# qiyu3816/DiffSG

Hardware: AMD Instinct MI355X
Metric: ddpm_reverse_sample_steps_per_sec_msr80c (higher is better)
Workload: dtype f32(2xf16-split MFMA, f32 accumulate); 1 GPU; MSR-80c CFG reverse sampling, batch 65536 x D=C=80 per GPU, UNet1D(proj 128, dims (64,32,16,8), n_blocks 2), omega=1, device Philox noise; rows sharded, no collective; batch_per_gpu=65536, solution_dim=80, parallelism=rows x1

## Files before the change

diffsg_amd/UNetCF.py:

```python
from __future__ import annotations

import ctypes

import torch
import torch.nn as nn

from . import _lib


class _ParamsOnly(nn.Module):
    def forward(self, *a, **k):
        raise RuntimeError("parameter holder: the arithmetic lives in libdiffsg_hip.so (call UNet1D.forward)")


class TimeEmbedding(_ParamsOnly):

    def __init__(self, in_dim):
        super().__init__()
        self.in_dim = in_dim
        self.lin1 = nn.Linear(in_dim // 4, in_dim)
        self.lin2 = nn.Linear(in_dim, in_dim)


class ResidualBlock(_ParamsOnly):
# ... 231 lines not shown
    def set_precision(self, mode):
        code = {"split_f16": 0, "f32": 1}[mode]
        for hd in self._all_handles():
            _lib.check(_lib.lib().dsg_set_precision(hd, code))
        self.__dict__.setdefault("_settings", {})["precision"] = code

    @property
    def precision(self):
        return {0: "split_f16", 1: "f32"}[self.__dict__.get("_settings", {}).get("precision", 0)]

    def range_exceeded(self):
        hit = False
        for nat in [self._native] + list(self.__dict__.get("_twins", {}).values()):
            hd = nat.handle
            if hd is None:
                continue
            flag = ctypes.c_int(0)
            with torch.cuda.device(self._named_param_list()[0][1].device):
                _lib.check(_lib.lib().dsg_range_status_stream(hd, ctypes.byref(flag), _lib.stream_ptr()))
            hit = hit or bool(flag.value)
        return hit

    def check_range(self):
        if self.range_exceeded():
            raise RuntimeError("libdiffsg_hip: an activation exceeded the fp16 range of the split-f16 path (|x| > 6e4); "
                               "the results of the last calls are invalid -- use set_precision('f32') for this model")

    def set_launch_policy(self, coop_max_tiles=-1, narrow_small_max_tiles=-1):
        for hd in self._all_handles():
            _lib.check(_lib.lib().dsg_set_launch_policy(hd, int(coop_max_tiles), int(narrow_small_max_tiles)))
        self.__dict__.setdefault("_settings", {})["policy"] = (int(coop_max_tiles), int(narrow_small_max_tiles))

    def set_option(self, name, value):
        code = {"narrow_valu8": 1, "train_time_beside": 2, "wgrad_narrow_part": 4, "tile_step": 8, "panel_half": 16, "f32_pair": 32}[name]
        for hd in self._all_handles():
            _lib.check(_lib.lib().dsg_set_option(hd, code, int(value)))
        self.__dict__.setdefault("_settings", {}).setdefault("options", {})[code] = int(value)

    def _all_handles(self):
        return [self.native_handle()] + [self.native_handle(k) for k in self.__dict__.get("_twins", {})]

    def forward(self, x, t, cond, cond_mask):
        hd = self.native_handle()
        B = x.shape[0]
        x = x.detach().to(torch.float32).contiguous()
        cond = cond.detach().to(torch.float32).contiguous()
        tv = t.detach().to(torch.float32).reshape(-1).contiguous()
        mk = cond_mask.detach().to(torch.float32).reshape(-1).contiguous()
        if tv.numel() != B or mk.numel() != B or cond.shape[0] != B:
            raise ValueError("t, cond and cond_mask must have one entry per row of x")
        if x.shape[1] != self.cfg["input_dim"] or cond.shape[1] != self.cfg["cond_dim"]:
            raise ValueError("x / cond feature size does not match the model")
        out = torch.empty_like(x)
        if B == 0:
            return out
        with torch.cuda.device(x.device):
            _lib.check(_lib.lib().dsg_unet_forward(hd, _lib.ptr(x), _lib.ptr(tv), _lib.ptr(cond), _lib.ptr(mk),
                                                   _lib.ptr(out), B, _lib.stream_ptr()))
        return out
```

diffsg_amd/csrc/dsg_api.hip:

```cpp
#include "dsg_kernels.hpp"
#include "dsg_train.hpp"
#include "dsg_split.hpp"
#include "dsg_wide.hpp"
#include "dsg_panel.hpp"
#include "dsg_res64.hpp"
#include "dsg_tile.hpp"
#include "dsg_train_split.hpp"
#include "dsg_eval.hpp"
#include "dsg_labelgen.hpp"
#include "dsg_cogen.hpp"
#include "dsg_nugen.hpp"
#include "../../include/diffsg.h"

#include <math.h>
#include <stdarg.h>
#include <stdio.h>
#include <string.h>

#include <string>
#include <algorithm>
#include <vector>

using namespace dsg;

// ... 141 lines not shown
    int device = 0;
    int* range_flag = nullptr;
    int* range_pinned = nullptr;
    CallParams* call_dev = nullptr;
    hipStream_t cap_stream = nullptr;
    std::vector<double> op_ms;
    bool train_prof = false;
    hipEvent_t tev[6] = {nullptr, nullptr, nullptr, nullptr, nullptr, nullptr};
    bool tev_valid = false;
    std::vector<int> op_calls;

    int fuse_lo = 0, fuse_hi = 0;
    FusedOp* fused_dev = nullptr;
    std::vector<FusedOp> fused_host;
    FusedOpH* fusedh_dev = nullptr;
    FusedOpH* tileops_dev = nullptr;
    std::vector<FusedOpH> tileops_host;
    bool tile_valid = false, opt_tile = true;
    bool opt_panel_half = true;
    FusedOpH* fusedh_train_dev = nullptr;
    const void* fusedh_train_key[4] = {nullptr, nullptr, nullptr, nullptr}; int fusedh_train_rows = 0;
    struct FusedSig { bool valid = false, sp = false, share = false; int nrows = 0, npass = 0, uncond_tiles = 0; const void* p[8] = {}; } fused_sig;
    FusedOp* ce_dev = nullptr;
    std::vector<FusedOp> ce_host;
    CondTile* ctile_dev = nullptr; int ctile_n = 0; const float* ctile_key = nullptr; size_t ctile_cap = 0;
    std::vector<FusedOpH> fusedh_host;
    NarrowLdsOp* nlds_ops_dev = nullptr; NarrowLdsCopy* nlds_copies_dev = nullptr; uint4* nlds_image = nullptr;
    std::vector<NarrowPhaseArgs> nlds_phases;
    bool nlds_tail = false;
    bool nlds_valid = false;
    int v8_lo = -1, v8_hi = -1;
    bool opt_v8 = true;
    bool opt_f32_pair = true;
    bool opt_time_beside = true;
    bool opt_wg_narrow_part = false;
    float* v8_image = nullptr; NarrowLdsCopy* v8_copies_dev = nullptr; int v8_ncopies = 0;
    int nlds_ncopies = 0;
    size_t nlds_image_cap = 0;

    hipGraphExec_t gexec[1 + 6] = {};
    int g_rows = -1, g_chunks = -1, g_chunk_rows = -1;
    unsigned long long* seeds_dev = nullptr; int seeds_cap = 0;
    double* red_chunks = nullptr; int red_chunks_cap = 0;

    size_t tr_per_tile = 0;
    size_t tr_yt_frag = 0, tr_deps = 0;
    int tr_rows = 0, tr_T = 0, tr_chunks = 0;
    float* tr_ws = nullptr;
    float* tr_slabs = nullptr;
    float* tr_gsum = nullptr;
    unsigned* tr_gmax = nullptr;
    unsigned* tr_gmax_t = nullptr;
    int gmax_ld = 0;
    float* tr_cs = nullptr;
    int4* cs_map_dev = nullptr;
    int cs_slots = 0;
    int n_gmax = 0;
    size_t slab_stride = 0;
    int* tr_ts = nullptr;
    float* tr_noise = nullptr; float* tr_mask = nullptr;
    float* tr_yt_rm = nullptr;
    float* tr_tsave = nullptr;
    long long* tw_dst_dev = nullptr; const float** tw_src_dev = nullptr; int tw_rows = 0;
    WgradDesc* wg_desc_dev = nullptr; WgradUnit* wg_unit_dev = nullptr; int wg_units = 0;
    std::vector<int> wg_forks = {3, 6};
    std::vector<int> wg_part_end;
// ... 396 lines not shown
    }
}

void fill_block_args_h(const dsg_handle* h, const ResP& r, const BlockArgs& b, BlockArgsH& a) {
    a.b = b;
    const float* A = h->arena;
    a.W1h = reinterpret_cast<const uint4*>(A + r.W1h); a.W2h = reinterpret_cast<const uint4*>(A + r.W2h);
    a.W3h = reinterpret_cast<const uint4*>(A + r.W3h); a.Wsch = r.sclin ? reinterpret_cast<const uint4*>(A + r.Wsch) : nullptr;
    a.m1 = h->maxabs + r.l1.w; a.m2 = h->maxabs + r.l2.w; a.m3 = h->maxabs + r.l3.w; a.msc = r.sclin ? h->maxabs + r.sc.w : nullptr;
    a.kc = h->opc_dev + 4 * (size_t)(&r - h->res.data());
}
void fill_lin_args_h(const dsg_handle* h, const LinOpP& l, const LinArgs& b, LinArgsH& a) {
    a.l = b;
    a.Wh = reinterpret_cast<const uint4*>(h->arena + l.Wh);
    a.m = h->maxabs + l.l.w;
    a.kc = h->opc_dev + 4 * (h->res.size() + (size_t)(&l - h->lin.data()));
}

template <int N>
void launch_res_h_n(bool sclin, const BlockArgsH& a, hipStream_t s) {
    const dim3 grid(cdiv(a.b.ntiles, kWavesPerBlock)), block(256);
    if (sclin) hipLaunchKernelGGL((k_resblock_h<N, true>), grid, block, 0, s, a);
    else hipLaunchKernelGGL((k_resblock_h<N, false>), grid, block, 0, s, a);
}

bool wide128_ok(const ResP& r, const BlockArgs& b) {
    return r.N == 128 && b.in0.groups == 16 && (b.in1.groups == 0 || b.in1.groups == 16) && (b.in1.groups != 0) == r.sclin && b.cond_pre;
}

bool panel128_ok(const dsg_handle* h, const ResP& r, const BlockArgs& b) {
    return wide128_ok(r, b) && !b.ts && !b.save_h1 && b.tiles_per_pass * 2 >= b.ntiles && b.ntiles >= h->panel_min_tiles &&
           b.ntiles > h->coop_max_tiles;
}
template <bool SC, int EPI, int NTO>
void launch_panel128(const dsg_handle* h, const BlockLinArgsH& w, hipStream_t s) {
    if (h->opt_panel_half) {
        const int ngroups = cdiv(w.b.b.ntiles, 4);
        const dim3 grid(ngroups < 2 * h->num_cus ? ngroups : 2 * h->num_cus), block(256);
        hipLaunchKernelGGL((k_panel128_h<SC, EPI, NTO, 2>), grid, block, 0, s, w, ngroups);
        return;
    }
    const int ngroups = cdiv(w.b.b.ntiles, kPW);
    const dim3 grid(ngroups < h->num_cus ? ngroups : h->num_cus), block(kPW * 64);
    hipLaunchKernelGGL((k_panel128_h<SC, EPI, NTO>), grid, block, 0, s, w, ngroups);
}

bool res64_lds_ok(const dsg_handle* h, const ResP& r, const BlockArgs& b) {
    return r.N == 64 && b.in0.groups == 8 && (b.in1.groups == 0 || b.in1.groups == 8) && (b.in1.groups != 0) == r.sclin && b.cond_pre && !b.ts &&
           !b.save_h1 && b.tiles_per_pass * 2 >= b.ntiles && b.ntiles >= h->panel_min_tiles && b.ntiles > h->coop_max_tiles;
}

void launch_res_h(const dsg_handle* h, const ResP& r, const BlockArgs& b, hipStream_t s) {
    BlockArgsH a;
    fill_block_args_h(h, r, b, a);
    const int ks1 = (groups_of(r.in0) + 1) / 2 + (groups_of(r.in1) + 1) / 2;
    const bool coop_fits = ks1 * 128 <= kCoopLdsU4 / (4 / (r.N / 32 > 0 ? r.N / 32 : 1)) / 2 && r.in0 == r.N && r.in1 == (r.sclin ? r.N : 0);
    const int coop_max = (a.b.save_h1 && h->coop_max_tiles > 0 && h->coop_max_tiles < kCoopMaxTilesTrain) ? kCoopMaxTilesTrain : h->coop_max_tiles;
    if ((r.N == 64 || r.N == 128) && coop_fits && a.b.ntiles <= coop_max) {
        const int tpw = 4 / (r.N / 32);
        const dim3 grid(cdiv(a.b.ntiles, tpw)), block(256);
        if (r.N == 128) {
            if (r.sclin) hipLaunchKernelGGL((k_resblock_c<128, true>), grid, block, 0, s, a);
            else hipLaunchKernelGGL((k_resblock_c<128, false>), grid, block, 0, s, a);
        } else {
            if (r.sclin) hipLaunchKernelGGL((k_resblock_c<64, true>), grid, block, 0, s, a);
            else hipLaunchKernelGGL((k_resblock_c<64, false>), grid, block, 0, s, a);
        }
        return;
    }
    if (res64_lds_ok(h, r, a.b)) {
        const int ngroups = cdiv(a.b.ntiles, kR64Waves);
        const dim3 grid(ngroups < h->num_cus ? ngroups : h->num_cus), block(kR64Waves * 64);
        BlockLinArgsH w;
        memset(&w, 0, sizeof w);
        w.b = a; w.store_block_out = 1;
        if (r.sclin) hipLaunchKernelGGL((k_res64_lds<true, 0>), grid, block, 0, s, w, ngroups);
        else hipLaunchKernelGGL((k_res64_lds<false, 0>), grid, block, 0, s, w, ngroups);
// ... 62 lines not shown
    }
    if (panel128_ok(h, r, b) && l.l.K == 128) {
#define DSG_TRYP(SC_, EPI_, NTO_)                                                                            \
    if (r.sclin == SC_ && (final_op ? 2 : 1) == EPI_ && NTO == NTO_) {                                       \
        launch_panel128<SC_, EPI_, NTO_>(h, a, s);                                                           \
        return true;                                                                                         \
    }
        DSG_TRYP(false, 1, 2) DSG_TRYP(false, 1, 1) DSG_TRYP(true, 2, 1) DSG_TRYP(true, 2, 3)
#undef DSG_TRYP
    }
    if (wide128_ok(r, b) && l.l.K == 128) {
#define DSG_TRYW(SC_, EPI_, NTO_)                                                                            \
    if (r.sclin == SC_ && (final_op ? 2 : 1) == EPI_ && NTO == NTO_) {                                       \
        hipLaunchKernelGGL((k_wide128_h<SC_, EPI_, NTO_>), grid, block, 0, s, a);                            \
        return true;                                                                                         \
    }
        DSG_TRYW(false, 1, 2) DSG_TRYW(false, 1, 1) DSG_TRYW(true, 2, 1) DSG_TRYW(true, 2, 3)
#undef DSG_TRYW
    }
#define DSG_TRY(N_, SC_, NTO_, FIN_)                                                                         \
    if (r.N == N_ && r.sclin == SC_ && NTO == NTO_ && final_op == FIN_) {                                    \
        hipLaunchKernelGGL((k_resblock_lin_h<N_, SC_, NTO_, FIN_>), grid, block, 0, s, a);                   \
        return true;                                                                                         \
    }
    DSG_TRY(128, false, 2, false) DSG_TRY(128, false, 1, false) DSG_TRY(64, true, 4, false) DSG_TRY(64, false, 2, false)
    DSG_TRY(64, true, 2, false) DSG_TRY(64, false, 1, false)
    DSG_TRY(128, true, 1, true) DSG_TRY(128, true, 3, true) DSG_TRY(64, true, 1, true) DSG_TRY(64, true, 3, true)
#undef DSG_TRY
    return false;
}

bool split_ctx(const dsg_handle* h, const RunCtx& c) { return h->use_split && c.cond_pre; }

void launch_op(const dsg_handle* h, const Op& op, const RunCtx& c, hipStream_t s) {
    if (op.kind == OP_RES) {
        BlockArgs a;
        fill_block_args(h, op, c, a);
        const ResP& r = h->res[op.p];
        if (split_ctx(h, c)) launch_res_h(h, r, a, s);
        else launch_res(r.N, r.sclin, a, s);
    } else {
        LinArgs a;
        fill_lin_args(h, op, c, a);
        const int inmode = op.kind == OP_PROJ ? IN_ROWMAJOR : IN_FRAG;
        const int outmode = op.kind == OP_FINAL ? OUT_ROWMAJOR : OUT_FRAG;
        if (split_ctx(h, c)) {
            LinArgsH ah;
            fill_lin_args_h(h, h->lin[op.p], a, ah);
            launch_lin_h(h->lin[op.p].l.N, inmode, outmode, op.kind == OP_FINAL, ah, s);
        } else {
            launch_lin(h->lin[op.p].l.N, inmode, outmode, op.kind == OP_FINAL, a, s);
        }
    }
}

bool fusable(const dsg_handle* h, const Op& op) {
    if (op.kind == OP_RES) return h->res[op.p].N <= 32;
    if (op.kind == OP_LIN) return h->lin[op.p].l.N <= 32;
    return false;
}

int prepare_fused(dsg_handle* h, const RunCtx& c, hipStream_t s) {
    const int n = h->fuse_hi - h->fuse_lo;
    if (n < 2) return 0;
    const bool sp = split_ctx(h, c);
    if (c.train) {
        if (!sp) return 0;
        const void* key[4] = {h->ws, h->tr_ws, h->cembed, h->tb};
        if (h->fusedh_train_dev && h->fusedh_train_rows == c.nrows && !memcmp(key, h->fusedh_train_key, sizeof key)) return 0;
        if (!h->fusedh_train_dev) HIPCK(hipMalloc(&h->fusedh_train_dev, (h->ops.size() + 1) * sizeof(FusedOpH)));
        memcpy(h->fusedh_train_key, key, sizeof key);
        h->fusedh_train_rows = c.nrows;
// ... 1169 lines not shown
    DeviceGuard dg(h);
    if (mode != DSG_PRECISION_SPLIT_F16 && mode != DSG_PRECISION_F32_MFMA) return fail("unknown precision mode %d", mode);
    const bool split = mode == DSG_PRECISION_SPLIT_F16;
    if (split != h->use_split) { (void)hipDeviceSynchronize(); free_graphs(h); h->use_split = split; }
    return 0;
}

int dsg_set_renorm_hook(dsg_handle* h, double* stats3, void (*reduce)(void*), void* user) {
    if (!h) return fail("null handle");
    if (reduce && !stats3) return fail("dsg_set_renorm_hook: a reduce function needs the 3-double device buffer");
    h->renorm_stats = stats3; h->renorm_fn = reduce; h->renorm_user = user;
    return 0;
}

int dsg_set_option(dsg_handle* h, int option, int value) {
    if (!h) return fail("null handle");
    DeviceGuard dg(h);
    switch (option) {
        case DSG_OPT_NARROW_VALU8:
            if ((value != 0) != h->opt_v8) {
                (void)hipDeviceSynchronize();
                free_graphs(h);
                h->fused_sig.valid = false;
                h->opt_v8 = value != 0;
            }
            return 0;
        case DSG_OPT_TRAIN_TIME_BESIDE: h->opt_time_beside = value != 0; return 0;
        case DSG_OPT_PANEL_HALF:
            if ((value != 0) != h->opt_panel_half) { (void)hipDeviceSynchronize(); free_graphs(h); h->opt_panel_half = value != 0; }
            return 0;
        case DSG_OPT_F32_PAIR:
            if ((value != 0) != h->opt_f32_pair) { (void)hipDeviceSynchronize(); free_graphs(h); h->opt_f32_pair = value != 0; }
            return 0;
        case DSG_OPT_TILE_STEP:
            if ((value != 0) != h->opt_tile) { (void)hipDeviceSynchronize(); free_graphs(h); h->opt_tile = value != 0; }
            return 0;
        case DSG_OPT_WGRAD_NARROW_PART:
            if ((value != 0) != h->opt_wg_narrow_part) { (void)hipDeviceSynchronize(); h->opt_wg_narrow_part = value != 0; h->td_valid = false; }
            return 0;
        default: return fail("dsg_set_option: unknown option %d", option);
    }
}

int dsg_range_status(dsg_handle* h, int* exceeded) {
    if (!h || !exceeded) return fail("dsg_range_status: null argument");
    DeviceGuard dg(h);
    HIPCK(hipDeviceSynchronize());
    HIPCK(hipMemcpy(exceeded, h->range_flag, sizeof(int), hipMemcpyDeviceToHost));
    if (*exceeded) HIPCK(hipMemset(h->range_flag, 0, sizeof(int)));
    return 0;
}

int dsg_range_status_stream(dsg_handle* h, int* exceeded, void* stream) {
    if (!h || !exceeded) return fail("dsg_range_status_stream: null argument");
    DeviceGuard dg(h);
    hipStream_t s = (hipStream_t)stream;
    if (!h->range_pinned) HIPCK(hipHostMalloc(reinterpret_cast<void**>(&h->range_pinned), sizeof(int), hipHostMallocDefault));
    hipLaunchKernelGGL(k_flag_take, dim3(1), dim3(64), 0, s, h->range_flag, h->range_pinned);
    HIPCK(hipGetLastError());
    HIPCK(hipStreamSynchronize(s));
    *exceeded = *h->range_pinned;
    return 0;
}

int dsg_set_launch_policy(dsg_handle* h, int coop_max_tiles, int narrow_small_max_tiles) {
    if (!h) return fail("null handle");
// ... 793 lines not shown
```

diffsg_amd/csrc/dsg_panel.hpp:

```cpp
#pragma once
#include "dsg_wide.hpp"

namespace dsg {

constexpr int kPW = 8;
constexpr int kPanelU4 = 2048;
constexpr int kPrivU4 = 128;
constexpr int kPrivSlots = 5;
constexpr int kPrivDist = 4;
constexpr int kPanelLdsU4 = 2 * kPanelU4 + kPW * kPrivSlots * kPrivU4 + kWideVec / 4;
constexpr int panel_pw(int steps) { return 2 * steps; }
constexpr int panel_u4(int steps) { return 512 * steps; }
constexpr int panel_lds_u4(int steps) { return 2 * panel_u4(steps) + panel_pw(steps) * kPrivSlots * kPrivU4 + kWideVec / 4; }

#ifndef DSG_STAMP_DBG
#define DSG_STAMP_DBG 0
#endif
#ifdef DSG_CYCLE_STAMPS
constexpr int kPanelStampU4 = kPW * 128 / 2;
#define DSG_PSTAMP(tag)                                                                                               \
    do {                                                                                                              \
        if (STAMPED && blockIdx.x == 0 && stamp_k < 128) {                                                           \
            const unsigned long long t_ = __builtin_readcyclecounter();                                               \
            if (lane == 0 && !(DSG_STAMP_DBG & 1)) stamp_lds[wave * 128 + stamp_k] = (t_ << 16) | (unsigned long long)(tag); \
// ... 216 lines not shown
        const int S = j < NJ ? S0 + 1 + j : nx.S, q = m & 3, tt = (S >> 1) & 3, r0 = 8 * (S & 1) + 2 * q, hs = m >> 1, e = 2 * (m & 1);
        const float dcur = j < NJ ? dd : ddn;
        if (ph == 0) {
            const float x0 = MEM ? xq[hs][e] : (j < NJ ? in[tt][r0] : (*nx.in)[tt][r0]), x1 = MEM ? xq[hs][e + 1] : (j < NJ ? in[tt][r0 + 1] : (*nx.in)[tt][r0 + 1]);
            if (LN) {
                u0 = fmaf(fmaf(x0, cp, dcur), gq[hs][e], bq[hs][e]);
                u1 = fmaf(fmaf(x1, cp, dcur), gq[hs][e + 1], bq[hs][e + 1]);
                p0 = __builtin_amdgcn_exp2f(u0); p1 = __builtin_amdgcn_exp2f(u1);
            } else {
                u0 = x0 * (cp * kRawScale); u1 = x1 * (cp * kRawScale);
            }
        } else if (ph == 1) {
            if (LN) {
                v0 = u0 * __builtin_amdgcn_rcpf(fmaf(p0, kk, kk));
                v1 = u1 * __builtin_amdgcn_rcpf(fmaf(p1, kk, kk));
            } else { v0 = u0; v1 = u1; }
        } else {
            unsigned a, er;
            split_pair_nowait(v0, v1, a, er);
            hq[m] = __builtin_bit_cast(float, a); lq[m] = __builtin_bit_cast(float, er);
        }
    }
    if (HASN) {
        constexpr int L0 = 4 * NJ;
        asm volatile("" : "+v"(hq[L0 + 3]), "+v"(lq[L0 + 3]));
        const f32x4 hv = {hq[L0], hq[L0 + 1], hq[L0 + 2], hq[L0 + 3]}, lv = {lq[L0], lq[L0 + 1], lq[L0 + 2], lq[L0 + 3]};
        bcarry.hi = __builtin_bit_cast(h8, hv); bcarry.lo = __builtin_bit_cast(h8, lv);
    }
}

#ifndef DSG_PANEL_TRAIL_PRIO
#define DSG_PANEL_TRAIL_PRIO 1
#endif
template <bool SCLIN, int EPI, int NTO, int STEPS = 4>
__global__ __launch_bounds__(64 * panel_pw(STEPS), 2) void k_panel128_h(const BlockLinArgsH A, const int ngroups) {
    constexpr int N = 128, NT = 4, NG = 16;
    constexpr int PW = panel_pw(STEPS), PU4 = panel_u4(STEPS), NTHR = 64 * PW;
    constexpr int KS1 = SCLIN ? 16 : 8, P1 = KS1 / STEPS, P2 = 8 / STEPS, NE = SCLIN ? 16 : 8;
    constexpr int NTOP = NTO <= 1 ? 1 : (NTO == 2 ? 2 : 4), ESTEPS = 4 * STEPS / NTOP;
    constexpr int EPANELS = EPI == 0 ? 0 : (ESTEPS >= 8 ? 1 : 8 / ESTEPS);
    constexpr int PA = P1, PB = PA + P2, PD = PB + P2, PE = PD + (SCLIN ? P1 : 0), NP = PE + EPANELS;
    __shared__ uint4 lds[panel_lds_u4(STEPS) + (STEPS == 4 ? kPanelStampU4 : 0)];
#ifdef DSG_CYCLE_STAMPS
    unsigned long long* const stamp_lds = reinterpret_cast<unsigned long long*>(lds + panel_lds_u4(STEPS));
    int stamp_k = 0;
    constexpr bool STAMPED = SCLIN && EPI == 0 && STEPS == 4;
#endif
    float* const vec = reinterpret_cast<float*>(lds + 2 * PU4 + PW * kPrivSlots * kPrivU4);
    float* const g1v = vec, * const b1v = vec + kLnLdsW1, * const v2 = vec + 2 * kLnLdsW1;
    float* const g2v = v2, * const b2v = v2 + 128, * const g3v = v2 + 256, * const b3v = v2 + 384, * const tbv = v2 + 512, * const c2v = v2 + 640,
         * const c3v = v2 + 768, * const gLv = v2 + 896, * const bLv = v2 + 1024, * const biasLv = v2 + 1152;
    const BlockArgsH& ah = A.b;
    const BlockArgs& a = ah.b;
    const int lane = threadIdx.x & 63, h = lane >> 5, j = lane & 31;
    const int wave = __builtin_amdgcn_readfirstlane(threadIdx.x >> 6);
    const int stride = gridDim.x;
#ifdef DSG_CYCLE_STAMPS
    const unsigned long long clk_t0 = __builtin_readcyclecounter(), clk_r0 = __builtin_amdgcn_s_memrealtime();
#endif
    const bool lead = wave < 4;
    if (STEPS == 4 && !lead) __builtin_amdgcn_s_setprio(DSG_PANEL_TRAIL_PRIO);
    constexpr float kL2 = -1.44269504088896341f;

    {
        const int n1 = ln1_extent(a);
        for (int i = threadIdx.x; i < n1; i += NTHR) { g1v[i] = a.gamma1[i] * kL2; b1v[i] = a.beta1[i] * kL2; }
        if (threadIdx.x < 128) {
            const int i = threadIdx.x;
            g2v[i] = a.gamma2[i] * kL2; b2v[i] = a.beta2[i] * kL2; g3v[i] = a.gamma3[i] * kL2; b3v[i] = a.beta3[i] * kL2;
            c2v[i] = a.c2[i]; c3v[i] = a.c3[i];
            tbv[i] = a.tbias[(size_t)(a.step_ptr ? *a.step_ptr : 0) * a.tb_stride + i];
            if (EPI == 2) { gLv[i] = A.l.l.gamma[i] * kL2; bLv[i] = A.l.l.beta[i] * kL2; }
            if (EPI != 0) biasLv[i] = i < NTO * 32 ? A.l.l.bias[i] : 0.f;
        }
    }
    const float inv1 = ah.kc[0], inv2 = ah.kc[1], inv3 = ah.kc[2];
    float invL = 0.f;
    if (EPI != 0) invL = A.l.kc[EPI == 2 ? 1 : 0];
    __syncthreads();

    const int wnt = wave / (STEPS / 2), wsub = wave % (STEPS / 2);
    const uint4* const w1p = ah.W1h + ((size_t)wnt * KS1) * 128 + wsub * 256;
    const uint4* const w2p = ah.W2h + ((size_t)wnt * 8) * 128 + wsub * 256;
    const uint4* const w3p = ah.W3h + ((size_t)wnt * 8) * 128 + wsub * 256;
    const uint4* const wsp = SCLIN ? ah.Wsch + ((size_t)wnt * KS1) * 128 + wsub * 256 : w1p;
    const uint4* wlp = w1p;
    if (EPI != 0) {
        if (NTOP == 4) wlp = A.l.Wh + ((size_t)(wnt < NTO ? wnt : 0) * 8) * 128 + wsub * 256;
        else if (NTOP == 2) wlp = A.l.Wh + ((size_t)(wave / STEPS) * 8) * 128 + (wave % STEPS) * 256;
        else wlp = A.l.Wh + (wave & 3) * 256;
    }
    auto panel_src = [&](int p) -> const uint4* {
        if (p < PA) return w1p + (size_t)p * (128 * STEPS);
        if (p < PB) return w2p + (size_t)(p - PA) * (128 * STEPS);
        if (p < PD) return w3p + (size_t)(p - PB) * (128 * STEPS);
        if (p < PE) return wsp + (size_t)(p - PD) * (128 * STEPS);
        return wlp + (ESTEPS < 8 ? (size_t)(p - PE) * (128 * ESTEPS) : 0);
    };

    const unsigned lds0 = (unsigned)(unsigned long long)(const __attribute__((address_space(3))) void*)lds;
    PanelCtx c;
    c.lane16 = (unsigned)lane * 16u; c.lane4 = (unsigned)lane * 4u;
    c.w_lds = lds0 + (unsigned)wave * 4096u;
    c.w_rd = lds0 + (unsigned)lane * 16u;
    c.p_lds = lds0 + 2u * PU4 * 16u + (unsigned)wave * (kPrivSlots * 2048u);
    c.wrd = lds + lane;
    c.prd = lds + 2 * PU4 + wave * (kPrivSlots * kPrivU4) + lane;
    c.q = 0; c.islot = 0; c.cslot = 0;

    {
        const TilePtrs cur = tile_ptrs<SCLIN, PW>(a, blockIdx.x < ngroups ? blockIdx.x : 0, wave);
        priv_issue_stats(c, cur.st0, cur.st1);
        priv_issue(c, cur.x0);
        priv_issue(c, cur.x0 + 2048);
        priv_issue(c, cur.x0 + 4096);
    }
    glds_quad_s(c.lane16, panel_src(0), c.w_lds);

    int since_w = 0;
    auto panel_begin = [&](int next) -> int {
        if (since_w >= 8) asm volatile("s_waitcnt vmcnt(8) lgkmcnt(0)" ::: "memory");
        else if (STEPS < 4 && since_w >= 4) asm volatile("s_waitcnt vmcnt(4) lgkmcnt(0)" ::: "memory");
        else if (since_w >= 2) asm volatile("s_waitcnt vmcnt(2) lgkmcnt(0)" ::: "memory");
        else asm volatile("s_waitcnt vmcnt(0) lgkmcnt(0)" ::: "memory");
        __builtin_amdgcn_s_barrier();
        const int rd = c.q & 1;
        glds_quad_s(c.lane16, panel_src(next), c.w_lds + (unsigned)((c.q + 1) & 1) * (PU4 * 16u));
        since_w = 0;
        ++c.q;
        return rd;
    };
    auto xin = [&](const TilePtrs& t, int S) -> const char* { return SCLIN && S >= 8 ? t.x1 + (size_t)(S - 8) * 2048 : t.x0 + (size_t)S * 2048; };

    constexpr bool XT = SCLIN && EPI == 0;
    BOp bcar;
    float cc_car = 0.f, dd_car = 0.f;
    for (int g = blockIdx.x; g < ngroups; g += stride) {
        const int tile_raw = g * PW + wave;
        const bool live = tile_raw < a.ntiles;
        const int tile = live ? tile_raw : a.ntiles - 1;
        const int ptile = tile >= a.tiles_per_pass ? tile - a.tiles_per_pass : tile;
        const TilePtrs cur = tile_ptrs<SCLIN, PW>(a, g, wave);
        const bool my_cond = cur.cond;
        const TilePtrs nxt = tile_ptrs<SCLIN, PW>(a, g + stride < ngroups ? g + stride : g, wave);
        DSG_PSTAMP(0x01);
        auto issue_tail = [&](int T) {
            if (T < NE) priv_issue(c, xin(cur, T));
            else if (T == NE) priv_issue_stats(c, nxt.st0, nxt.st1);
            else priv_issue(c, nxt.x0 + (size_t)(T - NE - 1) * 2048);
            since_w += 2;
        };
        auto consume_s1 = [&](int S) -> const uint4* {
            const uint4* rd = priv_consume(c);
            if (S + 4 < KS1) { priv_issue(c, xin(cur, S + 4)); since_w += 2; }
            else if (my_cond) { priv_issue(c, cur.cp + (size_t)(S + 4 - KS1) * 2048); since_w += 2; }
            else issue_tail(S + 4 - KS1);
            return rd;
        };
        auto consume_sc = [&](int S) -> const uint4* {
            const uint4* rd = priv_consume(c);
            issue_tail(S + 4);
            return rd;
        };
        auto no_consume = [&](int) -> const uint4* { return nullptr; };

        auto ln1_stats = [&](const TilePtrs& t, float& cc, float& dd) {
            const uint4* rd = priv_consume(c);
            const float2* sp = reinterpret_cast<const float2*>(rd - lane);
            const float2 s0 = sp[j];
            float mean = s0.x, m2 = s0.y;
            if (SCLIN) {
                const float2 s1 = sp[32 + j];
                const float dd_ = s1.x - mean;
                m2 = m2 + s1.y + dd_ * dd_ * a.chan_w;
                mean = mean + dd_ * a.chan_f;
            }
            priv_issue(c, t.x0 + 3 * 2048); since_w += 2;
            const float rstd = rsqrtf(m2 * a.inv_nin + kLnEps);
            if (SCLIN) range_check(a.range_flag, mean, m2);
            cc = rstd; dd = -mean * rstd;
        };

// ... 38 lines not shown
                }
                DSG_PSTAMP(0x12);
            }
        }
        acc_unscale_add_lds<NT>(acc1, inv1, tbv, h);
        DSG_PSTAMP(0x13);

        f32x16 acc2[NT];
        {
            float mean, m2;
            acc_stats<N, NT>(acc1, h, mean, m2);
            const float rstd = rsqrtf(m2 * (1.0f / N) + kLnEps), cc = rstd, dd = -mean * rstd;
            DSG_PSTAMP(0x20);
            BOp b0 = step0_reg(acc1, g2v, b2v, cc, dd), bc;
            asm volatile("" : "+v"(b0.hi), "+v"(b0.lo));
            DSG_PSTAMP(0x21);
#pragma unroll
            for (int p = 0; p < P2; ++p) {
                const int bi = panel_begin(PA + p + 1);
                DSG_PSTAMP(0x24);
                const NextPrep nx{&acc1, STEPS * (p + 1 < P2 ? p + 1 : 0), g2v, b2v, cc, dd, nullptr, nullptr};
                if (p + 1 < P2) {
                    if (p == 0) panel_pipe_s<true, PIPE_REG, PIPE_REG, STEPS>(acc2, c.wrd + bi * PU4, b0, bc, acc1, STEPS * p, g2v, b2v, cc, dd, h, no_consume, nx, none_n);
                    else panel_pipe_s<false, PIPE_REG, PIPE_REG, STEPS>(acc2, c.wrd + bi * PU4, b0, bc, acc1, STEPS * p, g2v, b2v, cc, dd, h, no_consume, nx, none_n);
                    b0 = bc;
                } else {
                    if (p == 0) panel_pipe_s<true, PIPE_REG, PIPE_NONE, STEPS>(acc2, c.wrd + bi * PU4, b0, bc, acc1, STEPS * p, g2v, b2v, cc, dd, h, no_consume, nx, none_n);
                    else panel_pipe_s<false, PIPE_REG, PIPE_NONE, STEPS>(acc2, c.wrd + bi * PU4, b0, bc, acc1, STEPS * p, g2v, b2v, cc, dd, h, no_consume, nx, none_n);
                }
                DSG_PSTAMP(0x22);
            }
            acc_unscale_add_lds<NT>(acc2, inv2, c2v, h);
        }
        if (my_cond) {
#pragma unroll
            for (int e = 0; e < 4; ++e) {
#pragma unroll
                for (int hf = 0; hf < 2; ++hf) {
                    const int i = 2 * e + hf;
                    const uint4* rd = priv_consume(c);
                    const float4 cv0 = __builtin_bit_cast(float4, rd[0]), cv1 = __builtin_bit_cast(float4, rd[64]);
                    if (i + 4 < 8) { priv_issue(c, cur.cp + (size_t)(i + 4) * 2048); since_w += 2; }
                    else issue_tail(i + 4 - 8);
                    const int r0 = 8 * hf;
                    acc2[e][r0 + 0] += cv0.x; acc2[e][r0 + 1] += cv0.y; acc2[e][r0 + 2] += cv0.z; acc2[e][r0 + 3] += cv0.w;
                    acc2[e][r0 + 4] += cv1.x; acc2[e][r0 + 5] += cv1.y; acc2[e][r0 + 6] += cv1.z; acc2[e][r0 + 7] += cv1.w;
                }
            }
        }
        DSG_PSTAMP(0x23);

        f32x16 (&acc3)[NT] = acc1;
        {
            float mean, m2;
            acc_stats<N, NT>(acc2, h, mean, m2);
            const float rstd = rsqrtf(m2 * (1.0f / N) + kLnEps), cc = rstd, dd = -mean * rstd;
            DSG_PSTAMP(0x30);
            BOp b0 = step0_reg(acc2, g3v, b3v, cc, dd), bc, bsc;
            asm volatile("" : "+v"(b0.hi), "+v"(b0.lo));
            DSG_PSTAMP(0x31);
            int bi = 0;
#pragma unroll
            for (int p = 0; p + 1 < P2; ++p) {
                bi = panel_begin(PB + p + 1);
                DSG_PSTAMP(0x34);
                const NextPrep nx{&acc2, STEPS * (p + 1), g3v, b3v, cc, dd, nullptr, nullptr};
                if (p == 0) panel_pipe_s<true, PIPE_REG, PIPE_REG, STEPS>(acc3, c.wrd + bi * PU4, b0, bc, acc2, STEPS * p, g3v, b3v, cc, dd, h, no_consume, nx, none_n);
                else panel_pipe_s<false, PIPE_REG, PIPE_REG, STEPS>(acc3, c.wrd + bi * PU4, b0, bc, acc2, STEPS * p, g3v, b3v, cc, dd, h, no_consume, nx, none_n);
                b0 = bc;
                DSG_PSTAMP(0x32);
            }
            bc = b0;
            constexpr int SL = 8 - STEPS;
            bi = panel_begin((PD) % NP);
            DSG_PSTAMP(0x34);
            if (SCLIN) {
                const NextPrep raw{&acc2, 0, g3v, b3v, 1.f, 0.f, nullptr, nullptr};
                panel_pipe_s<false, PIPE_REG, PIPE_RAW, STEPS>(acc3, c.wrd + bi * PU4, bc, bsc, acc2, SL, g3v, b3v, cc, dd, h, no_consume, raw,
                                                               [&]() { return consume_sc(0); });
                DSG_PSTAMP(0x32);
#pragma unroll
                for (int p = 0; p < P1; ++p) {
                    bi = panel_begin((PD + p + 1) % NP);
                    DSG_PSTAMP(0x44);
                    BOp bn;
                    auto cs = [&](int jj) { return consume_sc(STEPS * p + 1 + jj); };
                    if (p + 1 < P1) {
                        panel_pipe_s<false, PIPE_RAW, PIPE_RAW, STEPS>(acc3, c.wrd + bi * PU4, bsc, bn, acc3, STEPS * p, g3v, b3v, 1.f, 0.f, h, cs, raw,
                                                                       [&]() { return consume_sc(STEPS * p + STEPS); });
                        bsc = bn;
                    } else if (XT) {
                        const NextPrep nt1{&acc3, 0, g1v, b1v, 0.f, 0.f, &cc_car, &dd_car};
                        panel_pipe_s<false, PIPE_RAW, PIPE_LN, STEPS>(acc3, c.wrd + bi * PU4, bsc, bcar, acc3, STEPS * p, g3v, b3v, 1.f, 0.f, h, cs, nt1, [&]() {
                            ln1_stats(nxt, cc_car, dd_car);
                            const uint4* rd = priv_consume(c);
                            priv_issue(c, xin(nxt, 4)); since_w += 2;
                            return rd;
                        });
                    } else {
                        panel_pipe_s<false, PIPE_RAW, PIPE_NONE, STEPS>(acc3, c.wrd + bi * PU4, bsc, bn, acc3, STEPS * p, g3v, b3v, 1.f, 0.f, h, cs, raw, none_n);
                    }
                    DSG_PSTAMP(0x42);
                }
                acc_unscale_add_lds<NT>(acc3, inv3, c3v, h);
            } else {
                panel_pipe_s<false, PIPE_REG, PIPE_NONE, STEPS>(acc3, c.wrd + bi * PU4, bc, bsc, acc2, SL, g3v, b3v, cc, dd, h, no_consume,
                                                                NextPrep{&acc2, 0, g3v, b3v, cc, dd, nullptr, nullptr}, none_n);
                DSG_PSTAMP(0x32);
                acc_unscale_add_lds<NT>(acc3, inv3, c3v, h);
#pragma unroll
                for (int e = 0; e < 4; ++e) {
#pragma unroll
                    for (int hf = 0; hf < 2; ++hf) {
                        const int i = 2 * e + hf;
                        const uint4* rd = priv_consume(c);
                        const float4 xv0 = __builtin_bit_cast(float4, rd[0]), xv1 = __builtin_bit_cast(float4, rd[64]);
                        issue_tail(i + 4);
                        const int r0 = 8 * hf;
                        acc3[e][r0 + 0] += xv0.x; acc3[e][r0 + 1] += xv0.y; acc3[e][r0 + 2] += xv0.z; acc3[e][r0 + 3] += xv0.w;
                        acc3[e][r0 + 4] += xv1.x; acc3[e][r0 + 5] += xv1.y; acc3[e][r0 + 6] += xv1.z; acc3[e][r0 + 7] += xv1.w;
                    }
                }
            }
        }
        DSG_PSTAMP(0x43);

        float xmean, xm2;
        acc_stats<N, NT>(acc3, h, xmean, xm2);
        if ((EPI == 0 || A.store_block_out) && live) {
            if (h == 0) reinterpret_cast<float2*>(a.out_stats)[(size_t)tile * 32 + j] = make_float2(xmean, xm2);
#pragma unroll
            for (int G = 0; G < NG; ++G)
                st4(a.out + ((size_t)tile * NG + G) * 256 + lane * 4,
                    make_float4(acc3[G >> 2][4 * (G & 3)], acc3[G >> 2][4 * (G & 3) + 1], acc3[G >> 2][4 * (G & 3) + 2], acc3[G >> 2][4 * (G & 3) + 3]));
        }
        DSG_PSTAMP(0x50);
        if (EPI == 0) continue;
        if (EPI == 1) range_check(a.range_flag, xmean, xm2);

        const LinArgs& la = A.l.l;
        f32x16 acc[NTO];
        {
            const float cc = EPI == 2 ? rsqrtf(xm2 * la.inv_in_w + kLnEps) : 1.f, dd = -xmean * cc;
            const uint4* pn = nullptr;
#pragma unroll
            for (int S = 0; S < 8; ++S) {
                if (S % ESTEPS == 0) pn = c.wrd + panel_begin((PE + S / ESTEPS + 1) % NP) * PU4;
                const int sl = S % ESTEPS, t = S >> 1, r0 = 8 * (S & 1);
                HFrag<NTO> w;
                panel_wfrag<NTO>(w, pn, ESTEPS, sl);
                const float x[8] = {acc3[t][r0], acc3[t][r0 + 1], acc3[t][r0 + 2], acc3[t][r0 + 3], acc3[t][r0 + 4], acc3[t][r0 + 5], acc3[t][r0 + 6],
                                    acc3[t][r0 + 7]};
                float v[8];
                if (EPI == 2) {
                    const float4 g0 = ld4(gLv + 16 * S + 4 * h), b0 = ld4(bLv + 16 * S + 4 * h);
                    const float4 g1 = ld4(gLv + 16 * S + 8 + 4 * h), b1 = ld4(bLv + 16 * S + 8 + 4 * h);
                    act8_l2(v, x, cc, dd, g0, b0, g1, b1);
                } else {
#pragma unroll
                    for (int qq = 0; qq < 8; qq += 2) { const f32x2 tt = f32x2{x[qq], x[qq + 1]} * pk2(kRawScale); v[qq] = tt.x; v[qq + 1] = tt.y; }
                }
                h8 bhi, blo;
                split8(v, bhi, blo);
                if (S == 0) mfma_step_h0<NTO>(acc, w, bhi, blo); else mfma_step_h<NTO>(acc, w, bhi, blo);
            }
        }
// ... 14 lines not shown
            if (row < la.nrows) {
                float* o = la.out_rm + ((size_t)pass * la.nrows + row) * la.out_width;
                if ((la.out_width & 3) == 0) {
#pragma unroll
                    for (int G = 0; G < NTO * 4; ++G) {
                        const int f = 8 * G + 4 * h;
                        if (f < la.out_width)
                            st4(o + f, make_float4(acc[G >> 2][4 * (G & 3)], acc[G >> 2][4 * (G & 3) + 1], acc[G >> 2][4 * (G & 3) + 2], acc[G >> 2][4 * (G & 3) + 3]));
                    }
                } else {
#pragma unroll
                    for (int G = 0; G < NTO * 4; ++G)
#pragma unroll
                        for (int qq = 0; qq < 4; ++qq) {
                            const int f = 8 * G + 4 * h + qq;
                            if (f < la.out_width) o[f] = acc[G >> 2][4 * (G & 3) + qq];
                        }
                }
            }
        }
    }
    asm volatile("s_waitcnt vmcnt(0)" ::: "memory");
#ifdef DSG_CYCLE_STAMPS
    if (STAMPED && blockIdx.x == 0) {
        asm volatile("s_waitcnt lgkmcnt(0)" ::: "memory");
        for (int k = lane; k < 128; k += 64) dsg_stamp_buf[wave * 128 + k] = k < stamp_k ? stamp_lds[wave * 128 + k] : 0ull;
        if (threadIdx.x == 0) {
            dsg_stamp_buf[kPW * 128 + 0] = clk_t0; dsg_stamp_buf[kPW * 128 + 1] = clk_r0;
            dsg_stamp_buf[kPW * 128 + 2] = __builtin_readcyclecounter(); dsg_stamp_buf[kPW * 128 + 3] = __builtin_amdgcn_s_memrealtime();
            dsg_stamp_n = kPW * 128 + 4;
        }
    }
#endif
}

__global__ void k_calib_fill(uint4* __restrict__ p, size_t n) {
    for (size_t i = (size_t)blockIdx.x * 256 + threadIdx.x; i < n; i += (size_t)gridDim.x * 256) {
        unsigned hsh = (unsigned)i * 2654435761u;
        uint4 v;
        v.x = 0x38003800u | (hsh & 0x03ff03ffu); hsh = hsh * 1664525u + 1013904223u;
        v.y = 0x38003800u | (hsh & 0x03ff03ffu); hsh = hsh * 1664525u + 1013904223u;
        v.z = 0x38003800u | (hsh & 0x03ff03ffu); hsh = hsh * 1664525u + 1013904223u;
        v.w = 0x38003800u | (hsh & 0x03ff03ffu);
        p[i] = v;
    }
}

__global__ __launch_bounds__(512, 2) void k_calib_panel(const uint4* __restrict__ wbuf , const uint4* __restrict__ abuf,
                                                        size_t abuf_mask , int panels, float* __restrict__ sink) {
    __shared__ uint4 lds[2 * kPanelU4];
    const int lane = threadIdx.x & 63;
    const int wave = __builtin_amdgcn_readfirstlane(threadIdx.x >> 6);
    const unsigned lds0 = (unsigned)(unsigned long long)(const __attribute__((address_space(3))) void*)lds;
    const unsigned my = lds0 + (unsigned)wave * 4096u;
    typedef _Float16 h8c __attribute__((ext_vector_type(8)));
    h8c b;
#pragma unroll
    for (int i = 0; i < 8; ++i) b[i] = (_Float16)(-0.81f + 0.021f * (float)((threadIdx.x * 5 + i) & 31));
    f32x16 c[4] = {{0}, {0}, {0}, {0}};
    float v[12];
#pragma unroll
    for (int i = 0; i < 12; ++i) v[i] = 1.0f + 0.001f * (float)(threadIdx.x + i);
    for (int i = threadIdx.x; i < 2 * kPanelU4; i += 512) lds[i] = make_uint4(0x3c003c00u, 0x38003800u, 0x3a003a00u, 0x34003400u);
    __syncthreads();
    size_t apos = ((size_t)blockIdx.x * 8 + wave) * 128 + lane;
    const size_t astride = (size_t)gridDim.x * 8 * 128;
// ... 35 lines not shown
```

include/diffsg.h:

```cpp
#ifndef DIFFSG_H_
#define DIFFSG_H_

#ifdef __cplusplus
extern "C" {
#endif

typedef struct dsg_handle dsg_handle;

typedef struct {
    int input_dim;
    int proj_dim;
    int cond_dim;
    int n_res;
    int dims[8];
    int n_blocks;
} dsg_unet_desc;

dsg_handle* dsg_create(const dsg_unet_desc* desc);
void dsg_destroy(dsg_handle* h);
const char* dsg_last_error(void);
const char* dsg_build_id(void);

int dsg_param_count(const dsg_handle* h);
const char* dsg_param_name(const dsg_handle* h, int i);
long long dsg_param_numel(const dsg_handle* h, int i);
long long dsg_param_total(const dsg_handle* h);
int dsg_bind_weights(dsg_handle* h, const float* const* ptrs, int n, void* stream);

#define DSG_PRECISION_SPLIT_F16 0
#define DSG_PRECISION_F32_MFMA 1
int dsg_set_precision(dsg_handle* h, int mode);

int dsg_set_renorm_hook(dsg_handle* h, double* stats3, void (*reduce)(void* user), void* user);

int dsg_range_status(dsg_handle* h, int* exceeded);
int dsg_range_status_stream(dsg_handle* h, int* exceeded, void* stream);

int dsg_set_launch_policy(dsg_handle* h, int coop_max_tiles, int narrow_small_max_tiles);

enum { DSG_OPT_NARROW_VALU8 = 1, DSG_OPT_TRAIN_TIME_BESIDE = 2, DSG_OPT_WGRAD_NARROW_PART = 4, DSG_OPT_TILE_STEP = 8, DSG_OPT_PANEL_HALF = 16,
       DSG_OPT_F32_PAIR = 32 };
int dsg_set_option(dsg_handle* h, int option, int value);

int dsg_reserve(dsg_handle* h, int max_rows, int max_entries);

int dsg_unet_forward(dsg_handle* h, const float* x, const float* t, const float* cond, const float* cond_mask,
                     float* out, int B, void* stream);

#define DSG_SAMPLE_NO_GRAPH 1
#define DSG_SAMPLE_PROFILE 2
int dsg_sample(dsg_handle* h, const float* cond, const float* y_T, const float* noise, unsigned long long seed,
               float omega, const float* coef, int T, float* out, int B, int flags, void* stream);

int dsg_sample_rec(dsg_handle* h, const float* cond, const float* y_T, const float* noise, unsigned long long seed,
                   float omega, const float* coef, int T, float* out, int B, int flags, float* rec_y, float* rec_eps,
                   void* stream);

int dsg_sample_chunked(dsg_handle* h, const float* cond, const float* y_T, const float* noise, const unsigned long long* seeds,
                       int chunk_rows, float omega, const float* coef, int T, float* out, int B, int flags, void* stream);

int dsg_train_step(dsg_handle* h, const float* y, const float* cond, const int* ts, const float* noise,
                   const float* cond_mask, const float* sqrt_acp, const float* sqrt_1m_acp, int T, float* grads_flat,
                   float* loss_out, int B, void* stream);

int dsg_train_draws(unsigned long long seed, unsigned long long call, int T, float keep_prob, int B, int D, int* ts,
                    float* noise, float* cond_mask, void* stream);
int dsg_train_step_seeded(dsg_handle* h, const float* y, const float* cond, unsigned long long seed, unsigned long long call,
                          float keep_prob, const float* sqrt_acp, const float* sqrt_1m_acp, int T, float* grads_flat,
                          float* loss_out, int B, void* stream);

int dsg_train_profile_enable(dsg_handle* h, int on);
int dsg_train_profile(dsg_handle* h, float* ms5);

int dsg_adam_step(float* p, const float* g, float* exp_avg, float* exp_avg_sq, long long n, double lr, double beta1, double beta2, double eps,
// ... 38 lines not shown
```

Measured before the change: 1315 steps/s.

## Share first residual block stages between conditional and unconditional CFG passes

Adds a panel128 kernel variant for classifier-free guidance sampling. The first residual block runs its shared front half (stages 1-2) once per tile, writes the unconditional output, then adds the condition and finishes stage 3 again for the conditional pass. This avoids recomputing the identical pre-condition work and reloading the input for both CFG passes. In exchange it adds a longer tail prefetch schedule, extra weight panels and register pressure in the fused kernel, and it only applies under a narrow set of shape and flag conditions.

Result: no change. 1325 steps/s (median of 6 runs) (+0.7%).

```diff
diff --git a/diffsg_amd/UNetCF.py b/diffsg_amd/UNetCF.py
--- a/diffsg_amd/UNetCF.py
+++ b/diffsg_amd/UNetCF.py
@@ -287,7 +287,8 @@
         self.__dict__.setdefault("_settings", {})["policy"] = (int(coop_max_tiles), int(narrow_small_max_tiles))
 
     def set_option(self, name, value):
-        code = {"narrow_valu8": 1, "train_time_beside": 2, "wgrad_narrow_part": 4, "tile_step": 8, "panel_half": 16, "f32_pair": 32}[name]
+        code = {"narrow_valu8": 1, "train_time_beside": 2, "wgrad_narrow_part": 4, "tile_step": 8, "panel_half": 16, "f32_pair": 32,
+                "cfg_shared": 64}[name]
         for hd in self._all_handles():
             _lib.check(_lib.lib().dsg_set_option(hd, code, int(value)))
         self.__dict__.setdefault("_settings", {}).setdefault("options", {})[code] = int(value)
diff --git a/diffsg_amd/csrc/dsg_api.hip b/diffsg_amd/csrc/dsg_api.hip
--- a/diffsg_amd/csrc/dsg_api.hip
+++ b/diffsg_amd/csrc/dsg_api.hip
@@ -197,6 +197,7 @@
     int v8_lo = -1, v8_hi = -1;
     bool opt_v8 = true;
     bool opt_f32_pair = true;
+    bool opt_cfg_shared = true;
     bool opt_time_beside = true;
     bool opt_wg_narrow_part = false;
     float* v8_image = nullptr; NarrowLdsCopy* v8_copies_dev = nullptr; int v8_ncopies = 0;
@@ -659,17 +660,19 @@
     return wide128_ok(r, b) && !b.ts && !b.save_h1 && b.tiles_per_pass * 2 >= b.ntiles && b.ntiles >= h->panel_min_tiles &&
            b.ntiles > h->coop_max_tiles;
 }
-template <bool SC, int EPI, int NTO>
+template <bool SC, int EPI, int NTO, bool SHARED = false>
 void launch_panel128(const dsg_handle* h, const BlockLinArgsH& w, hipStream_t s) {
     if (h->opt_panel_half) {
         const int ngroups = cdiv(w.b.b.ntiles, 4);
         const dim3 grid(ngroups < 2 * h->num_cus ? ngroups : 2 * h->num_cus), block(256);
-        hipLaunchKernelGGL((k_panel128_h<SC, EPI, NTO, 2>), grid, block, 0, s, w, ngroups);
+        if (SHARED) hipLaunchKernelGGL((k_panel128_cfg_h<2>), grid, block, 0, s, w, ngroups);
+        else hipLaunchKernelGGL((k_panel128_h<SC, EPI, NTO, 2>), grid, block, 0, s, w, ngroups);
         return;
     }
     const int ngroups = cdiv(w.b.b.ntiles, kPW);
     const dim3 grid(ngroups < h->num_cus ? ngroups : h->num_cus), block(kPW * 64);
-    hipLaunchKernelGGL((k_panel128_h<SC, EPI, NTO>), grid, block, 0, s, w, ngroups);
+    if (SHARED) hipLaunchKernelGGL((k_panel128_cfg_h<4>), grid, block, 0, s, w, ngroups);
+    else hipLaunchKernelGGL((k_panel128_h<SC, EPI, NTO>), grid, block, 0, s, w, ngroups);
 }
 
 bool res64_lds_ok(const dsg_handle* h, const ResP& r, const BlockArgs& b) {
@@ -798,12 +801,24 @@
 
 bool split_ctx(const dsg_handle* h, const RunCtx& c) { return h->use_split && c.cond_pre; }
 
+bool cfg_shared_ok(const dsg_handle* h, const Op& op, const RunCtx& c, const ResP& r, const BlockArgs& b) {
+    return h->opt_cfg_shared && split_ctx(h, c) && c.share_proj && !c.train && c.npass == 2 && c.uncond_tiles == b.tiles_per_pass &&
+           op.in0 == h->ops[0].out && op.in1 < 0 && !r.sclin && b.in0.wrap == b.tiles_per_pass && panel128_ok(h, r, b);
+}
+
 void launch_op(const dsg_handle* h, const Op& op, const RunCtx& c, hipStream_t s) {
     if (op.kind == OP_RES) {
         BlockArgs a;
         fill_block_args(h, op, c, a);
         const ResP& r = h->res[op.p];
-        if (split_ctx(h, c)) launch_res_h(h, r, a, s);
+        if (cfg_shared_ok(h, op, c, r, a)) {
+            BlockLinArgsH w;
+            memset(&w, 0, sizeof w);
+            fill_block_args_h(h, r, a, w.b);
+            w.store_block_out = 1;
+            w.b.b.ntiles = a.tiles_per_pass;
+            launch_panel128<false, 0, 1, true>(h, w, s);
+        } else if (split_ctx(h, c)) launch_res_h(h, r, a, s);
         else launch_res(r.N, r.sclin, a, s);
     } else {
         LinArgs a;
@@ -2039,6 +2054,9 @@
         case DSG_OPT_F32_PAIR:
             if ((value != 0) != h->opt_f32_pair) { (void)hipDeviceSynchronize(); free_graphs(h); h->opt_f32_pair = value != 0; }
             return 0;
+        case DSG_OPT_CFG_SHARED:
+            if ((value != 0) != h->opt_cfg_shared) { (void)hipDeviceSynchronize(); free_graphs(h); h->opt_cfg_shared = value != 0; }
+            return 0;
         case DSG_OPT_TILE_STEP:
             if ((value != 0) != h->opt_tile) { (void)hipDeviceSynchronize(); free_graphs(h); h->opt_tile = value != 0; }
             return 0;
diff --git a/diffsg_amd/csrc/dsg_panel.hpp b/diffsg_amd/csrc/dsg_panel.hpp
--- a/diffsg_amd/csrc/dsg_panel.hpp
+++ b/diffsg_amd/csrc/dsg_panel.hpp
@@ -272,14 +272,16 @@
 #ifndef DSG_PANEL_TRAIL_PRIO
 #define DSG_PANEL_TRAIL_PRIO 1
 #endif
-template <bool SCLIN, int EPI, int NTO, int STEPS = 4>
-__global__ __launch_bounds__(64 * panel_pw(STEPS), 2) void k_panel128_h(const BlockLinArgsH A, const int ngroups) {
+template <bool SCLIN, int EPI, int NTO, int STEPS, bool SHARED>
+__device__ __attribute__((always_inline, flatten)) void panel128_body(const BlockLinArgsH A, const int ngroups) {
+    static_assert(!SHARED || (!SCLIN && EPI == 0), "the shared CFG head is an identity-shortcut block without an epilogue");
     constexpr int N = 128, NT = 4, NG = 16;
     constexpr int PW = panel_pw(STEPS), PU4 = panel_u4(STEPS), NTHR = 64 * PW;
     constexpr int KS1 = SCLIN ? 16 : 8, P1 = KS1 / STEPS, P2 = 8 / STEPS, NE = SCLIN ? 16 : 8;
+    constexpr int NTAIL = SHARED ? 3 * NE : NE;
     constexpr int NTOP = NTO <= 1 ? 1 : (NTO == 2 ? 2 : 4), ESTEPS = 4 * STEPS / NTOP;
     constexpr int EPANELS = EPI == 0 ? 0 : (ESTEPS >= 8 ? 1 : 8 / ESTEPS);
-    constexpr int PA = P1, PB = PA + P2, PD = PB + P2, PE = PD + (SCLIN ? P1 : 0), NP = PE + EPANELS;
+    constexpr int PA = P1, PB = PA + P2, PD = PB + P2, PE = PD + (SCLIN ? P1 : 0) + (SHARED ? P2 : 0), NP = PE + EPANELS;
     __shared__ uint4 lds[panel_lds_u4(STEPS) + (STEPS == 4 ? kPanelStampU4 : 0)];
 #ifdef DSG_CYCLE_STAMPS
     unsigned long long* const stamp_lds = reinterpret_cast<unsigned long long*>(lds + panel_lds_u4(STEPS));
@@ -334,7 +336,7 @@
         if (p < PA) return w1p + (size_t)p * (128 * STEPS);
         if (p < PB) return w2p + (size_t)(p - PA) * (128 * STEPS);
         if (p < PD) return w3p + (size_t)(p - PB) * (128 * STEPS);
-        if (p < PE) return wsp + (size_t)(p - PD) * (128 * STEPS);
+        if (p < PE) return (SHARED ? w3p : wsp) + (size_t)(p - PD) * (128 * STEPS);
         return wlp + (ESTEPS < 8 ? (size_t)(p - PE) * (128 * ESTEPS) : 0);
     };
 
@@ -386,8 +388,10 @@
         DSG_PSTAMP(0x01);
         auto issue_tail = [&](int T) {
             if (T < NE) priv_issue(c, xin(cur, T));
-            else if (T == NE) priv_issue_stats(c, nxt.st0, nxt.st1);
-            else priv_issue(c, nxt.x0 + (size_t)(T - NE - 1) * 2048);
+            else if (SHARED && T < 2 * NE) priv_issue(c, cur.cp + (size_t)(T - NE) * 2048);
+            else if (SHARED && T < 3 * NE) priv_issue(c, xin(cur, T - 2 * NE));
+            else if (T == NTAIL) priv_issue_stats(c, nxt.st0, nxt.st1);
+            else priv_issue(c, nxt.x0 + (size_t)(T - NTAIL - 1) * 2048);
             since_w += 2;
         };
         auto consume_s1 = [&](int S) -> const uint4* {
@@ -492,7 +496,7 @@
             }
             acc_unscale_add_lds<NT>(acc2, inv2, c2v, h);
         }
-        if (my_cond) {
+        auto add_cond = [&]() __attribute__((always_inline)) {
 #pragma unroll
             for (int e = 0; e < 4; ++e) {
 #pragma unroll
@@ -500,18 +504,20 @@
                     const int i = 2 * e + hf;
                     const uint4* rd = priv_consume(c);
                     const float4 cv0 = __builtin_bit_cast(float4, rd[0]), cv1 = __builtin_bit_cast(float4, rd[64]);
-                    if (i + 4 < 8) { priv_issue(c, cur.cp + (size_t)(i + 4) * 2048); since_w += 2; }
+                    if (SHARED) issue_tail(NE + i + 4);
+                    else if (i + 4 < 8) { priv_issue(c, cur.cp + (size_t)(i + 4) * 2048); since_w += 2; }
                     else issue_tail(i + 4 - 8);
                     const int r0 = 8 * hf;
                     acc2[e][r0 + 0] += cv0.x; acc2[e][r0 + 1] += cv0.y; acc2[e][r0 + 2] += cv0.z; acc2[e][r0 + 3] += cv0.w;
                     acc2[e][r0 + 4] += cv1.x; acc2[e][r0 + 5] += cv1.y; acc2[e][r0 + 6] += cv1.z; acc2[e][r0 + 7] += cv1.w;
                 }
             }
-        }
+        };
+        if (!SHARED && my_cond) add_cond();
         DSG_PSTAMP(0x23);
 
         f32x16 (&acc3)[NT] = acc1;
-        {
+        auto stage3 = [&](const int P3, const int PN, const int R0) __attribute__((always_inline)) {
             float mean, m2;
             acc_stats<N, NT>(acc2, h, mean, m2);
             const float rstd = rsqrtf(m2 * (1.0f / N) + kLnEps), cc = rstd, dd = -mean * rstd;
@@ -522,7 +528,7 @@
             int bi = 0;
 #pragma unroll
             for (int p = 0; p + 1 < P2; ++p) {
-                bi = panel_begin(PB + p + 1);
+                bi = panel_begin(P3 + p + 1);
                 DSG_PSTAMP(0x34);
                 const NextPrep nx{&acc2, STEPS * (p + 1), g3v, b3v, cc, dd, nullptr, nullptr};
                 if (p == 0) panel_pipe_s<true, PIPE_REG, PIPE_REG, STEPS>(acc3, c.wrd + bi * PU4, b0, bc, acc2, STEPS * p, g3v, b3v, cc, dd, h, no_consume, nx, none_n);
@@ -532,7 +538,7 @@
             }
             bc = b0;
             constexpr int SL = 8 - STEPS;
-            bi = panel_begin((PD) % NP);
+            bi = panel_begin(PN);
             DSG_PSTAMP(0x34);
             if (SCLIN) {
                 const NextPrep raw{&acc2, 0, g3v, b3v, 1.f, 0.f, nullptr, nullptr};
@@ -575,23 +581,43 @@
                         const int i = 2 * e + hf;
                         const uint4* rd = priv_consume(c);
                         const float4 xv0 = __builtin_bit_cast(float4, rd[0]), xv1 = __builtin_bit_cast(float4, rd[64]);
-                        issue_tail(i + 4);
+                        issue_tail(R0 + i + 4);
                         const int r0 = 8 * hf;
                         acc3[e][r0 + 0] += xv0.x; acc3[e][r0 + 1] += xv0.y; acc3[e][r0 + 2] += xv0.z; acc3[e][r0 + 3] += xv0.w;
                         acc3[e][r0 + 4] += xv1.x; acc3[e][r0 + 5] += xv1.y; acc3[e][r0 + 6] += xv1.z; acc3[e][r0 + 7] += xv1.w;
                     }
                 }
             }
-        }
-        DSG_PSTAMP(0x43);
-
+            DSG_PSTAMP(0x43);
+        };
+
+        if (SHARED) {
+            stage3(PB, PD, 0);
+            {
+                float m, m2;
+                acc_stats<N, NT>(acc3, h, m, m2);
+                if (live) {
+                    if (h == 0) reinterpret_cast<float2*>(a.out_stats)[(size_t)tile * 32 + j] = make_float2(m, m2);
+#pragma unroll
+                    for (int G = 0; G < NG; ++G)
+                        st4(a.out + ((size_t)tile * NG + G) * 256 + lane * 4,
+                            make_float4(acc3[G >> 2][4 * (G & 3)], acc3[G >> 2][4 * (G & 3) + 1], acc3[G >> 2][4 * (G & 3) + 2], acc3[G >> 2][4 * (G & 3) + 3]));
+                }
+            }
+            add_cond();
+            stage3(PD, 0, 2 * NE);
+        } else {
+            stage3(PB, PD % NP, 0);
+        }
+
+        const int otile = SHARED ? tile + a.tiles_per_pass : tile;
         float xmean, xm2;
         acc_stats<N, NT>(acc3, h, xmean, xm2);
         if ((EPI == 0 || A.store_block_out) && live) {
-            if (h == 0) reinterpret_cast<float2*>(a.out_stats)[(size_t)tile * 32 + j] = make_float2(xmean, xm2);
+            if (h == 0) reinterpret_cast<float2*>(a.out_stats)[(size_t)otile * 32 + j] = make_float2(xmean, xm2);
 #pragma unroll
             for (int G = 0; G < NG; ++G)
-                st4(a.out + ((size_t)tile * NG + G) * 256 + lane * 4,
+                st4(a.out + ((size_t)otile * NG + G) * 256 + lane * 4,
                     make_float4(acc3[G >> 2][4 * (G & 3)], acc3[G >> 2][4 * (G & 3) + 1], acc3[G >> 2][4 * (G & 3) + 2], acc3[G >> 2][4 * (G & 3) + 3]));
         }
         DSG_PSTAMP(0x50);
@@ -672,6 +698,15 @@
         }
     }
 #endif
+}
+
+template <bool SCLIN, int EPI, int NTO, int STEPS = 4>
+__global__ __launch_bounds__(64 * panel_pw(STEPS), 2) void k_panel128_h(const BlockLinArgsH A, const int ngroups) {
+    panel128_body<SCLIN, EPI, NTO, STEPS, false>(A, ngroups);
+}
+template <int STEPS = 4>
+__global__ __launch_bounds__(64 * panel_pw(STEPS), 2) void k_panel128_cfg_h(const BlockLinArgsH A, const int ngroups) {
+    panel128_body<false, 0, 1, STEPS, true>(A, ngroups);
 }
 
 __global__ void k_calib_fill(uint4* __restrict__ p, size_t n) {
diff --git a/include/diffsg.h b/include/diffsg.h
--- a/include/diffsg.h
+++ b/include/diffsg.h
@@ -39,7 +39,7 @@
 int dsg_set_launch_policy(dsg_handle* h, int coop_max_tiles, int narrow_small_max_tiles);
 
 enum { DSG_OPT_NARROW_VALU8 = 1, DSG_OPT_TRAIN_TIME_BESIDE = 2, DSG_OPT_WGRAD_NARROW_PART = 4, DSG_OPT_TILE_STEP = 8, DSG_OPT_PANEL_HALF = 16,
-       DSG_OPT_F32_PAIR = 32 };
+       DSG_OPT_F32_PAIR = 32, DSG_OPT_CFG_SHARED = 64 };
 int dsg_set_option(dsg_handle* h, int option, int value);
 
 int dsg_reserve(dsg_handle* h, int max_rows, int max_entries);
```
